# HDaoud/ORBSLAMM

Measured on AMD Instinct MI355X. Metric: frames/s ORB extract+match, 1241x376 @2000 kp; bit-exact kp/desc vs CPU, higher is better.
Workload: dtype u8

## Files before the change

### orbslamm_amd/csrc/orbx_geometry.inc

```

static int init_tables(orbx_handle* h)
{
    const OrbxParams& p = h->prm;
    if (p.nlevels < 1 || p.nlevels > ORBX_MAXL || p.nfeatures < 1 || !(p.scaleFactor > 1.0f))
        return fail(ORBX_E_INVALID, "bad ORBextractor parameters");
    const int L = p.nlevels;
    h->nlevels = L;
    const double scaleFactor = (double)p.scaleFactor;
    h->mvScaleFactor[0] = 1.0f;
    h->mvLevelSigma2[0] = 1.0f;
    for (int i = 1; i < L; i++) {
        h->mvScaleFactor[i] = (float)((double)h->mvScaleFactor[i - 1] * scaleFactor);
        h->mvLevelSigma2[i] = h->mvScaleFactor[i] * h->mvScaleFactor[i];
    }
    for (int i = 0; i < L; i++) {
        h->mvInvScaleFactor[i] = 1.0f / h->mvScaleFactor[i];
        h->mvInvLevelSigma2[i] = 1.0f / h->mvLevelSigma2[i];
    }
    const float factor = (float)(1.0 / scaleFactor);
    float nDesired = (float)p.nfeatures * (1 - factor) / (1 - (float)pow((double)factor, (double)L));
    int sum = 0;
    for (int l = 0; l < L - 1; l++) {
        h->mnFeaturesPerLevel[l] = cv_round(nDesired);
        sum += h->mnFeaturesPerLevel[l];
// ... 19 lines not shown
    Geom g;
    std::vector<Cell> cells;
    std::vector<short4> tabs;
    int xoff[ORBX_MAXL], yoff[ORBX_MAXL];
    int tileStrideDw, tileRows, fastListCap, tileRows0, fastListCap0, fastSmapPitch, fastSmapPitch0, nodeCap;
    BlurTiles bt;
    BlurRuns br;
    KpBlocks kb;
    int kbTotal;
    std::vector<PyrRange> pyrRanges;
    int pyrBlocks, pyrBufA, pyrBufB, pyrTabCap;
    bool pyrFused;
};

static inline size_t pyr_lds_bytes(int bufA, int bufB, int tabCap) { return ((size_t)bufA + bufB) * 4 + (size_t)tabCap * 16; }

static int build_geometry(const orbx_handle* h, int w, int h0, HostGeom& out)
{
    Geom& g = out.g;
    memset(&g, 0, sizeof g);
    g.nlevels = h->nlevels;
    g.w0 = w; g.h0 = h0;
    g.iniTh = h->prm.iniThFAST; g.minTh = h->prm.minThFAST;
    memcpy(g.umax, h->umax, sizeof g.umax);
    if (w > 8191 || h0 > 8191) return fail(ORBX_E_UNSUPPORTED, "frame larger than 8191 px");
    out.cells.clear();
    out.tabs.clear();
    int pyrOff = 0, blurOff = 0, candOff = 0, keptOff = 0, maxRoiW = 8, maxRoiH = 8, maxRoiW0 = 8, maxRoiH0 = 8, nodeCap = 16, maxCells = 1;
    for (int l = 0; l < g.nlevels; l++) {
        LevelGeom& L = g.lv[l];
// ... 249 lines not shown
```

### orbslamm_amd/csrc/orbx_kernels.hip

```cpp
#include <hip/hip_runtime.h>
#include <stdint.h>

#include "orbx_common.hpp"

namespace orbx {

struct FrameSrc {
    const uint8_t* img0;
    int32_t stride0;
    int64_t pitch0;
    uint8_t* pyr;
    uint8_t* blur;
    int32_t f0;
};

__device__ __forceinline__ const uint8_t* level_ptr(const Geom* g, const FrameSrc& s, int f, int l, int& stride)
{
    if (l == 0) { stride = s.stride0; return s.img0 + (int64_t)f * s.pitch0; }
    stride = g->lv[l].stride;
    return s.pyr + (int64_t)f * g->pyrFrameBytes + g->lv[l].pyrOff;
}

__device__ __forceinline__ bool xcd_block_frame(int nframes, int& blk, int& fr)
{
// ... 1551 lines not shown
constexpr DiscItems make_disc_items()
{
    DiscItems d{};
    int n = 0;
    for (int r = 0; r <= 2 * kDiscR; r++) {
        const int ay = r < kDiscR ? kDiscR - r : r - kDiscR, h = kDiscHalf[ay];
        for (int c = (kDiscR - h) / 4; c <= (kDiscR + h) / 4; c++) d.rc[n++] = (uint16_t)(r << 4 | c);
    }
    d.n = n;
    for (int t = n; t < kDiscLoads * 64; t++) d.rc[t] = d.rc[n - 1];
    return d;
}
__device__ const DiscItems kDisc = make_disc_items();
static_assert(make_disc_items().n <= kDiscLoads * 64 && make_disc_items().n > (kDiscLoads - 1) * 64, "five loads, not four");

__global__ __launch_bounds__(256) void k_orient_desc(const Geom* __restrict__ g, FrameSrc src, KpBlocks kb,
                                                    const uint64_t* __restrict__ kept,
                                                    const int32_t* __restrict__ keptCount,
                                                    OrbxKeyPointDev* __restrict__ outKps,
                                                    uint8_t* __restrict__ outDesc, int32_t* __restrict__ outCount, int nframes,
                                                    uint8_t* __restrict__ outX, int64_t xPitch, int64_t xAngOff)
{
#if ORBX_DESC_PRIO
    __builtin_amdgcn_s_setprio(ORBX_DESC_PRIO);
#endif
#ifdef ORBX_ORIENT_TIMING
    uint64_t ts[10]; int nts = 0;
#define OSTAMP() ts[nts++] = wall_clock64()
#else
#define OSTAMP() do {} while (0)
#endif
    OSTAMP();
    __shared__ float4 spat[256];
    __shared__ uint32_t swu[256], sw1[256];
    constexpr int PR = kDiscR, PDW = 10, PROWS = 2 * PR + 1;
    __shared__ uint32_t spatch[kKpPerBlock][PROWS * PDW];
    const int tid = threadIdx.x, lane = tid & 63, wave = tid >> 6;
    const int q = lane >> 4, ql = lane & 15;
    int bx, fr;
    if (!xcd_block_frame(nframes, bx, fr)) return;
    const int f = fr + src.f0;
    int l = 0;
    while (l + 1 < g->nlevels && bx >= kb.base[l + 1]) l++;
    const int idx = (bx - kb.base[l]) * kKpPerBlock + wave * 4 + q;
    const int nl = g->nlevels;
    const LevelGeom& L = g->lv[l];
    const uint64_t rec0 = kept[(int64_t)f * g->keptFrameRecs + L.keptOff + idx];
    int32_t pk = ((const int32_t*)d_pattern)[tid];
    const int tv = (tid >> 3) - kHalfPatch;
    int um = g->umax[(tv < 0 ? -tv : tv) & 15];
    int before = 0, totalAll = 0, mine = 0;
    for (int i = 0; i < nl; i++) {
        const int c = keptCount[f * nl + i];
        if (i < l) before += c;
        if (i == l) mine = c;
        totalAll += c;
    }
    if (bx == 0 && tid == 0) outCount[f] = totalAll < g->maxKp ? totalAll : g->maxKp;
    int ditem[kDiscLoads];
#pragma unroll
    for (int i = 0; i < kDiscLoads; i++) ditem[i] = kDisc.rc[64 * i + lane];
    asm volatile("" : "+v"(pk), "+v"(um), "+v"(ditem[0]), "+v"(ditem[1]), "+v"(ditem[2]), "+v"(ditem[3]), "+v"(ditem[4]));
    static_assert(kDiscLoads == 5, "operand list above");
    const int o = before + idx;
    const bool active = idx < mine && o < g->maxKp;
    const bool anyActive = __builtin_amdgcn_ballot_w64(active) != 0;
    OSTAMP();
    const uint64_t rec = active ? rec0 : 0;
    const int cx = (int)cand_x(rec) + kMinBorder, cy = (int)cand_y(rec) + kMinBorder;
    int stride;
    const uint8_t* img = level_ptr(g, src, f, l, stride);
    const int bs = L.blurStride;
    const uint8_t* blur = src.blur + (int64_t)f * g->blurFrameBytes + L.blurOff;
    const int ctrOff = cy * stride + cx, bctrOff = cy * bs + cx;

    OSTAMP();
    uint32_t dw[4][4];
    if (anyActive) {
        const uint32_t voff = (uint32_t)((lane >> 3) * stride + 4 * (lane & 7));
#pragma unroll
        for (int k = 0; k < 4; k++) {
            const uint8_t* pk = img + (__builtin_amdgcn_readlane(ctrOff, 16 * k) - kHalfPatch * stride - 16);
#pragma unroll
            for (int j = 0; j < 4; j++) gload_sbase(dw[k][j], voff, pk + 8 * j * stride);
        }
    }
    constexpr int NPI = kDiscLoads;
    uint32_t pd[4][NPI];
    int sidx[NPI];
    if (anyActive) {
        uint32_t voff[NPI];
#pragma unroll
        for (int i = 0; i < NPI; i++) {
            const int it = ditem[i], r = it >> 4, c = it & 15;
            voff[i] = (uint32_t)(r * bs + 4 * c);
            sidx[i] = r * PDW + c;
        }
#pragma unroll
        for (int k = 0; k < 4; k++) {
            const int so = __builtin_amdgcn_readlane((int)active, 16 * k) ? __builtin_amdgcn_readlane(bctrOff, 16 * k) : __builtin_amdgcn_readlane(bctrOff, 0);
            const uint8_t* pk = blur + (so - PR * bs - PR);
#pragma unroll
            for (int i = 0; i < NPI; i++) gload_sbase(pd[k][i], voff[i], pk);
        }
    }
    {
        spat[tid] = make_float4((float)(int8_t)(pk & 0xFF), (float)(int8_t)((pk >> 8) & 0xFF),
                                (float)(int8_t)((pk >> 16) & 0xFF), (float)(int8_t)((pk >> 24) & 0xFF));
        const int u0 = 4 * (tid & 7) - 16;
        const int d = tid < 248 ? um : -1;
        uint32_t wu = 0, w1 = 0;
#pragma unroll
        for (int j = 0; j < 4; j++) {
            const int u = u0 + j;
            if (u >= -d && u <= d) { wu |= (uint32_t)(u + 16) << (8 * j); w1 |= 1u << (8 * j); }
        }
        swu[tid] = wu; sw1[tid] = w1;
    }
    __syncthreads();
    if (!anyActive) return;
    OSTAMP();
    int m10, m01;
    asm volatile("s_waitcnt vmcnt(20)"
                 : "+v"(dw[0][0]), "+v"(dw[0][1]), "+v"(dw[0][2]), "+v"(dw[0][3]), "+v"(dw[1][0]), "+v"(dw[1][1]), "+v"(dw[1][2]), "+v"(dw[1][3]),
                   "+v"(dw[2][0]), "+v"(dw[2][1]), "+v"(dw[2][2]), "+v"(dw[2][3]), "+v"(dw[3][0]), "+v"(dw[3][1]), "+v"(dw[3][2]), "+v"(dw[3][3]));
    static_assert(4 * NPI == 20, "vmcnt above");
    {
        int A[4], B[4];
        uint32_t wu[4], w1[4], wv[4];
#pragma unroll
        for (int j = 0; j < 4; j++) {
            wu[j] = swu[lane + 64 * j];
            w1[j] = sw1[lane + 64 * j];
            wv[j] = w1[j] * (uint32_t)(8 * j + (lane >> 3) + 1);
        }
#pragma unroll
        for (int k = 0; k < 4; k++) {
            uint32_t su = 0, sv = 0, s1 = 0;
#pragma unroll
            for (int j = 0; j < 4; j++) {
                su = __builtin_amdgcn_udot4(dw[k][j], wu[j], su, false);
                sv = __builtin_amdgcn_udot4(dw[k][j], wv[j], sv, false);
                s1 = __builtin_amdgcn_udot4(dw[k][j], w1[j], s1, false);
            }
            A[k] = (int)su - 16 * (int)s1;
            B[k] = (int)sv - 16 * (int)s1;
        }
        auto swap32 = [](int a, int b) { const auto r = __builtin_amdgcn_permlane32_swap((unsigned)a, (unsigned)b, false, false); return (int)(r[0] + r[1]); };
        auto swap16 = [](int a, int b) { const auto r = __builtin_amdgcn_permlane16_swap((unsigned)a, (unsigned)b, false, false); return (int)(r[0] + r[1]); };
        m10 = swap16(swap32(A[0], A[2]), swap32(A[1], A[3]));
        m01 = swap16(swap32(B[0], B[2]), swap32(B[1], B[3]));
        m10 += __builtin_amdgcn_update_dpp(0, m10, 0x128, 0xF, 0xF, false);
        m01 += __builtin_amdgcn_update_dpp(0, m01, 0x128, 0xF, 0xF, false);
        m10 += __builtin_amdgcn_update_dpp(0, m10, 0x124, 0xF, 0xF, false);
        m01 += __builtin_amdgcn_update_dpp(0, m01, 0x124, 0xF, 0xF, false);
        m10 += __builtin_amdgcn_update_dpp(0, m10, 0x122, 0xF, 0xF, false);
        m01 += __builtin_amdgcn_update_dpp(0, m01, 0x122, 0xF, 0xF, false);
        m10 += __builtin_amdgcn_update_dpp(0, m10, 0x121, 0xF, 0xF, false);
        m01 += __builtin_amdgcn_update_dpp(0, m01, 0x121, 0xF, 0xF, false);
    }
    OSTAMP();
    asm volatile("s_waitcnt vmcnt(0)"
                 : "+v"(pd[0][0]), "+v"(pd[0][1]), "+v"(pd[0][2]), "+v"(pd[0][3]), "+v"(pd[0][4]),
                   "+v"(pd[1][0]), "+v"(pd[1][1]), "+v"(pd[1][2]), "+v"(pd[1][3]), "+v"(pd[1][4]),
                   "+v"(pd[2][0]), "+v"(pd[2][1]), "+v"(pd[2][2]), "+v"(pd[2][3]), "+v"(pd[2][4]),
                   "+v"(pd[3][0]), "+v"(pd[3][1]), "+v"(pd[3][2]), "+v"(pd[3][3]), "+v"(pd[3][4]));
    static_assert(NPI == 5, "operand list above");
#pragma unroll
    for (int k = 0; k < 4; k++)
#pragma unroll
        for (int i = 0; i < NPI; i++) spatch[wave * 4 + k][sidx[i]] = pd[k][i];
    const float angle = fast_atan2_deg((float)m01, (float)m10);

    constexpr float factorPI = (float)(3.1415926535897932384626433832795 / 180.f);
    const float ang = __fmul_rn(angle, factorPI);
    float a, b;
    orbx_sincosf_0_2pi(ang, &b, &a);
    OSTAMP();
    const uint8_t* const sp8 = (const uint8_t*)&spatch[0][0];
    constexpr float kRnd = 12582912.f;
    const uint32_t adj = (uint32_t)((wave * 4 + q) * (PROWS * PDW * 4) + PR * (PDW * 4) + PR) - 0x400000u * (uint32_t)(PDW * 4) - 0x4B400000u;
    static_assert(PDW * 4 == 40, "row pitch is an inline constant of the mad below");
    uint32_t myWord = 0;
    typedef float f2v __attribute__((ext_vector_type(2)));
    const f2v AB = {a, b}, KR = {kRnd, kRnd};
    auto rot = [&](const f2v p, int& rx, int& ry) {
        f2v U, V, W, Z;
        asm("v_pk_mul_f32 %0, %1, %2 op_sel:[0,0] op_sel_hi:[0,1]" : "=v"(U) : "v"(p), "v"(AB));
        asm("v_pk_mul_f32 %0, %1, %2 op_sel:[1,1] op_sel_hi:[1,0] neg_lo:[0,1]" : "=v"(V) : "v"(p), "v"(AB));
        asm("v_pk_add_f32 %0, %1, %2" : "=v"(W) : "v"(U), "v"(V));
        asm("v_pk_add_f32 %0, %1, %2" : "=v"(Z) : "v"(W), "v"(KR));
        rx = __float_as_int(Z.x); ry = __float_as_int(Z.y);
    };
#pragma unroll
    for (int t = 0; t < 16; t++) {
        const float4 pt = spat[ql + 16 * t];
        int rx0, ry0, rx1, ry1;
        rot(f2v{pt.x, pt.y}, rx0, ry0);
        rot(f2v{pt.z, pt.w}, rx1, ry1);
        uint32_t o0, o1;
        asm("v_mad_i32_i24 %0, %1, 40, %2" : "=v"(o0) : "v"(ry0), "v"(rx0));
        asm("v_mad_i32_i24 %0, %1, 40, %2" : "=v"(o1) : "v"(ry1), "v"(rx1));
        const int t0 = sp8[o0 + adj], t1 = sp8[o1 + adj];
        const uint64_t bal = __builtin_amdgcn_ballot_w64(t0 < t1);
        const uint32_t w16 = (uint32_t)(bal >> (16 * q)) & 0xFFFFu;
        if (ql == t) myWord = w16;
    }
    OSTAMP();
#ifdef ORBX_ORIENT_TIMING
    if (lane == 0 && wave == 0 && fr == 0 && (bx % 29) == 0)
        printf("ORIENT bx %d l %d: barrier %.2f counts %.2f rec %.2f moments %.2f trig %.2f brief %.2f us\n", bx, l, (ts[1]-ts[0])/100.0, (ts[2]-ts[1])/100.0, (ts[3]-ts[2])/100.0, (ts[4]-ts[3])/100.0, (ts[5]-ts[4])/100.0, (ts[6]-ts[5])/100.0);
#endif
    if (outX) {
        uint16_t* const sw = (uint16_t*)&spatch[wave * 4 + q][0];
        sw[ql] = (uint16_t)myWord;
        __builtin_amdgcn_fence(__ATOMIC_RELEASE, "wavefront");
        __builtin_amdgcn_wave_barrier();
        __builtin_amdgcn_fence(__ATOMIC_ACQUIRE, "wavefront");
        const int kq = (lane >> 3) & 3, c = lane & 7;
        const int oq = __shfl(o, 16 * kq);
        const bool aq = __shfl((int)active, 16 * kq) != 0;
        if (lane < 32 && aq) {
            const uint32_t bits = spatch[wave * 4 + kq][c];
            auto pm1 = [](uint32_t b8) {
                uint32_t x = (b8 | (b8 << 12)) & 0x000F000Fu;
                x = (x | (x << 6)) & 0x03030303u;
                x = (x | (x << 3)) & 0x11111111u;
                return 0x22222222u | ((x ^ 0x11111111u) << 3);
            };
            const uint4 e = make_uint4(pm1(bits & 255), pm1((bits >> 8) & 255), pm1((bits >> 16) & 255), pm1(bits >> 24));
            *(uint4*)(outX + (int64_t)f * xPitch + (int64_t)(oq >> 5) * 4096 + (int64_t)(c * 32 + (oq & 31)) * 16) = e;
        }
    }
    if (active) {
        ((uint16_t*)(outDesc + ((int64_t)f * g->maxKp + o) * 32))[ql] = (uint16_t)myWord;
        if (ql == 1 && outX) *(float*)(outX + (int64_t)f * xPitch + xAngOff + (int64_t)o * 4) = angle;
        if (ql == 0) {
            OrbxKeyPointDev kp;
            kp.x = __fmul_rn((float)cx, L.scale);
            kp.y = __fmul_rn((float)cy, L.scale);
            kp.size = L.kpSize;
            kp.angle = angle;
            kp.response = (float)cand_resp(rec);
            kp.octave = l;
            kp.class_id = -1;
            outKps[(int64_t)f * g->maxKp + o] = kp;
        }
    }
}

__global__ __launch_bounds__(256) void k_upload(const uint4* __restrict__ src, uint4* __restrict__ dst, int n16)
{
    typedef unsigned int u32x4 __attribute__((ext_vector_type(4)));
    const int i = blockIdx.x * 256 + threadIdx.x;
    if (i < n16) ((u32x4*)dst)[i] = __builtin_nontemporal_load((const u32x4*)src + i);
}

struct UploadSrcs { const uint4* src[8]; };
__global__ __launch_bounds__(256) void k_upload_frames(UploadSrcs s, uint4* __restrict__ dst, int n16)
{
    typedef unsigned int u32x4 __attribute__((ext_vector_type(4)));
    const int i = blockIdx.x * 256 + threadIdx.x, f = blockIdx.y;
// ... 220 lines not shown
```

### orbslamm_amd/csrc/orbx_pipeline.inc

```

static int configure_shape(orbx_handle* h, int w, int hh)
{
    if (h->curW == w && h->curH == hh) return ORBX_OK;
    if (w > h->maxW || hh > h->maxH) return fail(ORBX_E_INVALID, "frame %dx%d exceeds the handle's maximum %dx%d", w, hh, h->maxW, h->maxH);
    HostGeom hg;
    int rc = build_geometry(h, w, hh, hg);
    if (rc) return rc;
    if (hg.cells.size() > h->cellsCap || hg.tabs.size() > h->tabsCap || (size_t)hg.g.pyrFrameBytes > h->pyrCapFrame ||
        (size_t)hg.g.blurFrameBytes > h->blurCapFrame || (size_t)hg.g.candFrameRecs > h->candCapFrame ||
        (size_t)hg.g.keptFrameRecs > h->keptCapFrame || hg.g.maxKp > h->maxKp)
        return fail(ORBX_E_INVALID, "frame %dx%d needs more scratch than the handle was created with", w, hh);
    const size_t dl = dist_lds_bytes(hg.nodeCap, hg.g.maxCellsPerLevel);
    h->distInLds = dl <= 156 * 1024;
    if (h->distInLds && dl > 48 * 1024 &&
        hipFuncSetAttribute((const void*)k_distribute<true>, hipFuncAttributeMaxDynamicSharedMemorySize, (int)dl) != hipSuccess) {
        (void)hipGetLastError();
        h->distInLds = false;
    }
    if (h->distInLds) {
        h->distBlurOk = hipFuncSetAttribute((const void*)k_distribute_blur, hipFuncAttributeMaxDynamicSharedMemorySize, (int)dl) == hipSuccess;
        if (!h->distBlurOk) (void)hipGetLastError();
    } else {
        const size_t need = dl * (size_t)h->maxB * hg.g.nlevels;
        if (need > h->distScratchBytes && ((rc = sync_all(h)) || (rc = regrow_exact(h->d_distScratch, h->distScratchBytes, need, need)))) return rc;
// ... 102 lines not shown
        if (!h->distInLds || !h->distBlurOk || h->prof.cur || src.f0 != 0) return false;
        const size_t dl = dist_lds_bytes(h->nodeCap, g.maxCellsPerLevel);
        const int nTiles = h->blurTiles.base[g.nlevels];
        DistArgs da{h->d_geom, h->d_candRaw, h->d_candA, h->d_candB, h->d_cells, h->d_cellCount, h->d_candCount, h->d_kept, h->d_keptCount,
                    h->d_errCur, h->nodeCap, src.f0, nullptr, 0, 0};
        hipLaunchKernelGGL(k_distribute_blur, dim3(g.nlevels + (nTiles + 1) / 2, nb), dim3(kDistThreads), dl, s, da, src, h->blurTiles, nTiles);
        return true;
    }
    void blur(hipStream_t s, bool lat = false) const
    {
        h->prof.begin(P_BLUR, s);
        if (lat) hipLaunchKernelGGL(k_blur_mfma, dim3(h->blurTiles.base[h->geom.nlevels], xcd_grid_y(nb)), dim3(256), 0, s, h->d_geom, src, h->blurTiles, nb);
        else hipLaunchKernelGGL(k_blur_walk, dim3(h->blurRuns.base[h->geom.nlevels], xcd_grid_y(nb)), dim3(256), 0, s, h->d_geom, src, h->blurRuns, nb);
        h->prof.end(s);
    }
    int desc(hipStream_t s, int set, hipEvent_t done = nullptr) const
    {
        if (h->matchPending[set] && h->matchStream[set] != s) HIPCHK(hipStreamWaitEvent(s, h->evMatch[set], 0));
        if (h->evOutOfSet[set] && h->outStream[set] != s) HIPCHK(hipStreamWaitEvent(s, h->evOutOfSet[set], 0));
        for (hipEvent_t e : h->evExtReader[set]) HIPCHK(hipStreamWaitEvent(s, e, 0));
        h->evExtReader[set].clear();
        uint8_t* const xOut = h->fuseExpand ? r_xdesc(h, set) + (size_t)h->xPitch : nullptr;
        return launch_done(h, P_ORIENT_DESC, k_orient_desc, dim3(h->kpBlocksTotal, xcd_grid_y(nb)), dim3(256), 0, s, done, h->d_geom, src, h->kpBlocks, h->d_kept,
                           h->d_keptCount, r_kps(h, set) + h->maxKp, r_desc(h, set) + (size_t)h->maxKp * 32, r_count(h, set) + 1, nb, xOut, h->xPitch, h->xAngOff);
    }
};

struct FrameRange { int f0, f1; };
static inline FrameRange part_range(int B, int part, int nparts) { return {(int)((int64_t)B * part / nparts), (int)((int64_t)B * (part + 1) / nparts)}; }
struct CallMode { bool lat; int parts; };
static inline CallMode call_mode(const orbx_handle* h, int B)
{
    const bool lat = B <= h->latMaxB && !h->serial;
    return {lat, lat || h->serial ? 1 : std::min(h->nsplit, B)};
}

static int run_extract(orbx_handle* h, const uint8_t* d_imgs, int B, int w, int hh, int stride, size_t pitch,
                       const hipEvent_t* evUploaded = nullptr, hipStream_t sIn = nullptr, bool lazyDone = false)
{
// ... 44 lines not shown
            }
        } else {
            if (evFrames && sIn != sm) HIPCHK(hipStreamWaitEvent(sm, evFrames, 0));
            if (evFrames && sIn != sa) HIPCHK(hipStreamWaitEvent(sa, evFrames, 0));
            if (sIn == sa && h->partEverRan[0]) { if ((rc = flush_part_event(h))) return rc; HIPCHK(hipStreamWaitEvent(sa, h->evPart[0], 0)); }
            L.fast(sa, 0, cellsL0);
            L.dist(sa, 0, 1);
            if ((rc = L.pyramid(sm, h->evPyr[0]))) return rc;
            L.fast(sm, cellsL0, g.totalCells - cellsL0);
            L.dist(sm, 1, g.nlevels - 1);
            HIPCHK(hipStreamWaitEvent(sa, h->evPyr[0], 0));
            L.blur(sa, true);
            HIPCHK(hipEventRecord(h->evFast0[0], sa));
            HIPCHK(hipStreamWaitEvent(sm, h->evFast0[0], 0));
        }
        if ((rc = L.desc(sm, set, lazyDone ? nullptr : h->evPart[0]))) return rc;
        h->lastParts = 1; h->partLazy = lazyDone; h->partEverRan[0] = true;
    } else {
        for (int part = 0; part < nsplit; part++) {
            const FrameRange fr = part_range(B, part, nsplit);
            const int f0 = fr.f0, nb = fr.f1 - fr.f0;
            if (nb <= 0) continue;
            hipStream_t s = h->serial ? s0 : h->streamP[part];
            hipStream_t s2 = h->serial ? s : s0;
            if (evUploaded) {
                HIPCHK(hipStreamWaitEvent(s, evUploaded[part], 0));
                if (s2 != s) HIPCHK(hipStreamWaitEvent(s2, evUploaded[part], 0));
            }
            if (evFrames && !h->serial) HIPCHK(hipStreamWaitEvent(s, evFrames, 0));
            if (evFrames && !h->serial && sIn != s0 && part == 0) HIPCHK(hipStreamWaitEvent(s0, evFrames, 0));
            src.f0 = f0;
// ... 3 lines not shown
                if (h->partEverRan[part]) HIPCHK(hipStreamWaitEvent(s2, h->evPart[part], 0));
                L.fast(s2, 0, cellsL0);
                HIPCHK(hipEventRecord(h->evFast0[part], s2));
            } else {
                L.fast(s, 0, cellsL0);
            }
            if ((rc = L.pyramid(s))) return rc;
            HIPCHK(hipEventRecord(h->evPyr[part], s));
            HIPCHK(hipStreamWaitEvent(s2, h->evPyr[part], 0));
            L.blur(s2, B <= h->latMaxB);
            HIPCHK(hipEventRecord(h->evBlur[part], s2));
            L.fast(s, cellsL0, g.totalCells - cellsL0);
            if (splitFast) HIPCHK(hipStreamWaitEvent(s, h->evFast0[part], 0));
            L.dist(s, 0, g.nlevels);
            HIPCHK(hipStreamWaitEvent(s, h->evBlur[part], 0));
            if ((rc = L.desc(s, set))) return rc;
            HIPCHK(hipEventRecord(h->evPart[h->lastParts++], s));
            h->partEverRan[part] = true;
        }
    }
    HIPCHK(hipGetLastError());
    h->lastB = B;
    src.f0 = 0;
    h->lastSrc = src;
    return ORBX_OK;
}

extern "C" int orbx_extract_batch_device(orbx_t* h, const uint8_t* d_imgs, int B, int w, int hh, int stride, size_t pitch)
{
    int rc = check_device(h);
    if (rc) return rc;
// ... 81 lines not shown
```

### orbslamm_amd/csrc/orbx_probe.inc

```

extern "C" int orbx_compute_stereo_matches(orbx_t* left, orbx_t* right, int frame, float mb, float mbf,
                                           float* u_right, float* depth, int cap, int* n_left)
{
    int rc = orbx_sync(right);
    if (rc) return rc;
    if ((rc = orbx_sync(left))) return rc;
    if (left->device != right->device) return fail(ORBX_E_INVALID, "the two extractors live on different devices");
    if (left->curW == 0 || left->curW != right->curW || left->curH != right->curH || left->nlevels != right->nlevels)
        return fail(ORBX_E_INVALID, "left and right frames differ in shape or pyramid");
    if (frame < 0 || frame >= left->lastB || frame >= right->lastB) return fail(ORBX_E_INVALID, "frame %d not in the last batches", frame);
    if (!(mb > 0.f) || !(mbf > 0.f)) return fail(ORBX_E_INVALID, "stereo baseline (mb, mbf) must be positive");
    if (left->maxKp >= 65536 || right->maxKp >= 65536) return fail(ORBX_E_UNSUPPORTED, "more than 65535 keypoints per frame");
    int32_t n = 0;
    HIPCHK(hipMemcpy(&n, r_count(left, left->curSet) + 1 + frame, sizeof n, hipMemcpyDeviceToHost));
    if (n_left) *n_left = n;
    if (n > cap) return fail(ORBX_E_CAPACITY, "%d keypoints, caller capacity %d", n, cap);
    if (n == 0) return ORBX_OK;
    const size_t need = (size_t)left->maxKp * 12 + 64;
    if (need > left->stereoBytes && (rc = regrow_exact(left->d_stereo, left->stereoBytes, need, need))) return rc;
    StereoArgs a;
    a.kL = r_kps(left, left->curSet) + (size_t)(frame + 1) * left->maxKp; a.dL = r_desc(left, left->curSet) + (size_t)(frame + 1) * left->maxKp * 32;
    a.nL = r_count(left, left->curSet) + 1 + frame;
    a.kR = r_kps(right, right->curSet) + (size_t)(frame + 1) * right->maxKp; a.dR = r_desc(right, right->curSet) + (size_t)(frame + 1) * right->maxKp * 32;
    a.nR = r_count(right, right->curSet) + 1 + frame;
// ... 180 lines not shown
    auto launch = [&](int k, hipStream_t s) {
        switch (k) {
        case 0: (void)L.pyramid(s); break;
        case 1: L.fast(s, 0, cellsL0); L.fast(s, cellsL0, g.totalCells - cellsL0); break;
        case 2: L.dist(s, 0, g.nlevels); break;
        case 3: L.blur(s); break;
        case 4: (void)L.desc(s, set); break;
        default: match_kernels(h, s, set, nb, 0.7f, 50, 1); break;
        }
    };
    if (lds_bytes && wg_threads && wgs) {
        const size_t pl = pyr_lds_bytes(h->pyrBufA, h->pyrBufB, h->pyrTabCap);
        const size_t fl = fast_lds_bytes(h->tileRows, h->tileStrideDw, h->fastSmapPitch, h->fastListCap);
        const int nqb = (h->maxKp + orbm::kMfmaRowsPerBlock - 1) / orbm::kMfmaRowsPerBlock;
        const int32_t l[K] = {(int32_t)pl, (int32_t)fl, (int32_t)(dist_lds_bytes(h->nodeCap, g.maxCellsPerLevel) + 5552), (kBlurWalkInWords + kBlurMfmaOutWords) * 4, 31104, orbm::kMfmaLdsBytes};
        const int32_t t[K] = {256, 64, kDistThreads, 256, 256, 256};
        const int32_t w[K] = {h->pyrBlocks * nb, g.totalCells * nb, g.nlevels * nb, h->blurRuns.base[g.nlevels] * nb, h->kpBlocksTotal * nb, nqb * nb};
        for (int k = 0; k < K; k++) { lds_bytes[k] = l[k]; wg_threads[k] = t[k]; wgs[k] = w[k]; }
    }
    for (int k = 0; k < K; k++) if (names) names[k] = kNames[k];
    hipStream_t sa = h->streamP[0], sb = h->streamP[1];
    hipEvent_t e0, e1, eGo;
    HIPCHK(hipEventCreate(&e0)); HIPCHK(hipEventCreate(&e1)); HIPCHK(hipEventCreateWithFlags(&eGo, hipEventDisableTiming));
    auto timed = [&](int i, int j, int ni, int nj, float& ms) -> int {
        HIPCHK(hipEventRecord(eGo, h->stream));
        HIPCHK(hipStreamWaitEvent(sa, eGo, 0));
        if (j >= 0) { HIPCHK(hipStreamWaitEvent(sb, eGo, 0)); for (int r = 0; r < nj / 4; r++) launch(j, sb); }
        HIPCHK(hipEventRecord(e0, sa));
        for (int r = 0; r < ni; r++) { launch(i, sa); if (j >= 0) for (int q = 0; q * ni < nj - nj / 4 && q < 8; q++) launch(j, sb); }
        HIPCHK(hipEventRecord(e1, sa));
        HIPCHK(hipStreamSynchronize(sa)); HIPCHK(hipStreamSynchronize(sb));
// ... 24 lines not shown
```

### orbslamm_amd/csrc/orbx_streams.inc

```

struct ChainPool { hipStream_t s[4] = {nullptr, nullptr, nullptr, nullptr}; int users[4] = {0, 0, 0, 0}; bool made = false; };
static ChainPool g_chain[64];
static std::mutex g_chainMu;

static bool chain_prio_normal() { static const bool v = env_char("ORBX_LAT_PRIO") == '0'; return v; }

static int chain_stream_acquire(int device, int priority, hipStream_t* out, int* idx)
{
    std::lock_guard<std::mutex> lk(g_chainMu);
    ChainPool& cp = g_chain[device & 63];
    if (!cp.made) {
        hipStream_t s[4] = {nullptr, nullptr, nullptr, nullptr};
        void* scratch = nullptr;
        hipError_t e = hipMalloc(&scratch, 256);
        for (int i = 0; i < 4 && e == hipSuccess; i++) e = hipStreamCreateWithPriority(&s[i], hipStreamNonBlocking, priority);
        for (int i = 0; i < 4 && e == hipSuccess; i++) { e = hipMemsetAsync(scratch, 0, 256, s[i]); if (e == hipSuccess) e = hipStreamSynchronize(s[i]); }
        if (scratch) (void)hipFree(scratch);
        if (e != hipSuccess) {
            for (hipStream_t st : s) if (st) (void)hipStreamDestroy(st);
            return fail(ORBX_E_HIP, "cannot make the chain streams of device %d: %s", device, hipGetErrorString(e));
        }
        for (int i = 0; i < 4; i++) cp.s[i] = s[i];
        cp.made = true;
    }
// ... 160 lines not shown
        HIPCHK_OR(new_event(h, h->evBlur[i]), undo());
        HIPCHK_OR(new_event(h, h->evPart[i]), undo());
        HIPCHK_OR(new_event(h, h->evFast0[i]), undo());
    }
    HIPCHK_OR(new_event(h, h->evStart), undo());
    for (int i = 0; i < 2; i++) { HIPCHK_OR(new_event(h, h->evMatch[i]), undo()); HIPCHK_OR(new_event(h, h->evMatched[i]), undo()); }
    const size_t B = (size_t)max_batch;
    h->cellsCap = hg.cells.size() * 2 + 64;
    h->tabsCap = hg.tabs.size() * 2 + 64;
    h->imgFrameBytes = (size_t)align_up(max_w, 64) * max_h;
    h->pyrCapFrame = (size_t)hg.g.pyrFrameBytes + 4096;
    h->blurCapFrame = (size_t)hg.g.blurFrameBytes + 4096;
    h->candCapFrame = (size_t)hg.g.candFrameRecs + 1024;
    h->keptCapFrame = (size_t)hg.g.keptFrameRecs + 64;
    h->maxKp = hg.g.maxKp + 64;
    HIPCHK_OR(dev_alloc(h, h->d_geom, sizeof(Geom)), undo());
    HIPCHK_OR(dev_alloc(h, h->d_cells, h->cellsCap * sizeof(Cell)), undo());
    HIPCHK_OR(dev_alloc(h, h->d_tabs, h->tabsCap * sizeof(short4)), undo());
    h->pyrRangesCap = 64 * ORBX_MAXL;
    HIPCHK_OR(hipMalloc(&h->d_pyrRanges, h->pyrRangesCap * sizeof(PyrRange)), undo());
    HIPCHK_OR(dev_alloc(h, h->d_pyr, h->pyrCapFrame * B), undo());
    HIPCHK_OR(dev_alloc(h, h->d_blur, h->blurCapFrame * B), undo());
    HIPCHK_OR(dev_alloc(h, h->d_candRaw, h->candCapFrame * B * sizeof(uint64_t)), undo());
    HIPCHK_OR(dev_alloc(h, h->d_candA, h->candCapFrame * B * sizeof(uint64_t)), undo());
    HIPCHK_OR(dev_alloc(h, h->d_candB, h->candCapFrame * B * sizeof(uint64_t)), undo());
    HIPCHK_OR(dev_alloc(h, h->d_candCount, B * ORBX_MAXL * sizeof(int32_t)), undo());
    HIPCHK_OR(dev_alloc(h, h->d_cellCount, B * h->cellsCap * sizeof(int32_t)), undo());
    HIPCHK_OR(dev_alloc(h, h->d_kept, h->keptCapFrame * B * sizeof(uint64_t)), undo());
    HIPCHK_OR(dev_alloc(h, h->d_keptCount, B * ORBX_MAXL * sizeof(int32_t)), undo());
    HIPCHK_OR(dev_alloc(h, h->d_err, 8 * sizeof(int32_t)), undo());
    HIPCHK_OR(dev_alloc(h, h->d_kps, 2 * (B + 1) * h->maxKp * sizeof(OrbxKeyPointDev)), undo());
// ... 78 lines not shown
```

Before: 188,700.

## Template orient/desc kernel to process eight keypoints per wave for batched paths

```diff
diff --git a/orbslamm_amd/csrc/orbx_geometry.inc b/orbslamm_amd/csrc/orbx_geometry.inc
--- a/orbslamm_amd/csrc/orbx_geometry.inc
+++ b/orbslamm_amd/csrc/orbx_geometry.inc
@@ -57,6 +57,24 @@
 };
 
 static inline size_t pyr_lds_bytes(int bufA, int bufB, int tabCap) { return ((size_t)bufA + bufB) * 4 + (size_t)tabCap * 16; }
+
+static const int8_t kPatternHost[1024] = {
+#include "brief_pattern.inc"
+};
+static void build_orient_tables(const int umax[16], OrientTables& t)
+{
+    for (int i = 0; i < 256; i++) {
+        t.spat[i] = make_float4((float)kPatternHost[4 * i], (float)kPatternHost[4 * i + 1], (float)kPatternHost[4 * i + 2], (float)kPatternHost[4 * i + 3]);
+        const int v = (i >> 3) - kHalfPatch, u0 = 4 * (i & 7) - 16;
+        const int d = i < 248 ? umax[(v < 0 ? -v : v) & 15] : -1;
+        uint32_t wu = 0, w1 = 0;
+        for (int j = 0; j < 4; j++) {
+            const int u = u0 + j;
+            if (u >= -d && u <= d) { wu |= (uint32_t)(u + 16) << (8 * j); w1 |= 1u << (8 * j); }
+        }
+        t.swu[i] = wu; t.sw1[i] = w1;
+    }
+}
 
 static int build_geometry(const orbx_handle* h, int w, int h0, HostGeom& out)
 {
diff --git a/orbslamm_amd/csrc/orbx_kernels.hip b/orbslamm_amd/csrc/orbx_kernels.hip
--- a/orbslamm_amd/csrc/orbx_kernels.hip
+++ b/orbslamm_amd/csrc/orbx_kernels.hip
@@ -1589,13 +1589,22 @@
 __device__ const DiscItems kDisc = make_disc_items();
 static_assert(make_disc_items().n <= kDiscLoads * 64 && make_disc_items().n > (kDiscLoads - 1) * 64, "five loads, not four");
 
-__global__ __launch_bounds__(256) void k_orient_desc(const Geom* __restrict__ g, FrameSrc src, KpBlocks kb,
+struct OrientTables { float4 spat[256]; uint32_t swu[256], sw1[256]; };
+static_assert(sizeof(Geom) % 16 == 0 && sizeof(OrientTables) == 6144, "the tables follow the Geom block, 16-byte aligned");
+__device__ __forceinline__ const OrientTables* orient_tables(const Geom* g) { return (const OrientTables*)(g + 1); }
+
+template <int KPW>
+__global__ __launch_bounds__(kKpPerBlock / KPW * 64) void k_orient_desc(const Geom* __restrict__ g, FrameSrc src, KpBlocks kb,
                                                     const uint64_t* __restrict__ kept,
                                                     const int32_t* __restrict__ keptCount,
                                                     OrbxKeyPointDev* __restrict__ outKps,
                                                     uint8_t* __restrict__ outDesc, int32_t* __restrict__ outCount, int nframes,
                                                     uint8_t* __restrict__ outX, int64_t xPitch, int64_t xAngOff)
 {
+    static_assert(KPW == 4 || KPW == 8, "a quarter or an eighth of the wave per keypoint");
+    constexpr int EL = 64 / KPW, ELSH = KPW == 4 ? 4 : 3;
+    constexpr int NT = kKpPerBlock / KPW * 64;
+    static_assert(NT == 256 || (KPW == 8 && NT == 128), "the tables' 256 entries are built by 256 threads, or copied by 128 or 256");
 #if ORBX_DESC_PRIO
     __builtin_amdgcn_s_setprio(ORBX_DESC_PRIO);
 #endif
@@ -1611,19 +1620,34 @@
     constexpr int PR = kDiscR, PDW = 10, PROWS = 2 * PR + 1;
     __shared__ uint32_t spatch[kKpPerBlock][PROWS * PDW];
     const int tid = threadIdx.x, lane = tid & 63, wave = tid >> 6;
-    const int q = lane >> 4, ql = lane & 15;
+    const int q = lane >> ELSH, ql = lane & (EL - 1);
     int bx, fr;
     if (!xcd_block_frame(nframes, bx, fr)) return;
     const int f = fr + src.f0;
     int l = 0;
     while (l + 1 < g->nlevels && bx >= kb.base[l + 1]) l++;
-    const int idx = (bx - kb.base[l]) * kKpPerBlock + wave * 4 + q;
+    const int idx = (bx - kb.base[l]) * kKpPerBlock + wave * KPW + q;
     const int nl = g->nlevels;
     const LevelGeom& L = g->lv[l];
     const uint64_t rec0 = kept[(int64_t)f * g->keptFrameRecs + L.keptOff + idx];
-    int32_t pk = ((const int32_t*)d_pattern)[tid];
-    const int tv = (tid >> 3) - kHalfPatch;
-    int um = g->umax[(tv < 0 ? -tv : tv) & 15];
+    int32_t pk = 0;
+    int um = 0;
+    float4 tp0, tp1;
+    uint2 twu, tw1;
+    if constexpr (KPW == 4) {
+        pk = ((const int32_t*)d_pattern)[tid];
+        const int tv = (tid >> 3) - kHalfPatch;
+        um = g->umax[(tv < 0 ? -tv : tv) & 15];
+    } else {
+        const OrientTables* const T = orient_tables(g);
+        if constexpr (NT == 128) {
+            tp0 = T->spat[tid]; tp1 = T->spat[tid + 128];
+            twu = ((const uint2*)T->swu)[tid]; tw1 = ((const uint2*)T->sw1)[tid];
+        } else {
+            tp0 = tp1 = T->spat[tid];
+            twu.x = twu.y = T->swu[tid]; tw1.x = tw1.y = T->sw1[tid];
+        }
+    }
     int before = 0, totalAll = 0, mine = 0;
     for (int i = 0; i < nl; i++) {
         const int c = keptCount[f * nl + i];
@@ -1635,8 +1659,14 @@
     int ditem[kDiscLoads];
 #pragma unroll
     for (int i = 0; i < kDiscLoads; i++) ditem[i] = kDisc.rc[64 * i + lane];
-    asm volatile("" : "+v"(pk), "+v"(um), "+v"(ditem[0]), "+v"(ditem[1]), "+v"(ditem[2]), "+v"(ditem[3]), "+v"(ditem[4]));
-    static_assert(kDiscLoads == 5, "operand list above");
+    if constexpr (KPW == 4) {
+        asm volatile("" : "+v"(pk), "+v"(um), "+v"(ditem[0]), "+v"(ditem[1]), "+v"(ditem[2]), "+v"(ditem[3]), "+v"(ditem[4]));
+    } else {
+        asm volatile("" : "+v"(tp0.x), "+v"(tp0.y), "+v"(tp0.z), "+v"(tp0.w), "+v"(tp1.x), "+v"(tp1.y), "+v"(tp1.z), "+v"(tp1.w),
+                          "+v"(twu.x), "+v"(twu.y), "+v"(tw1.x), "+v"(tw1.y),
+                          "+v"(ditem[0]), "+v"(ditem[1]), "+v"(ditem[2]), "+v"(ditem[3]), "+v"(ditem[4]));
+    }
+    static_assert(kDiscLoads == 5, "operand lists above");
     const int o = before + idx;
     const bool active = idx < mine && o < g->maxKp;
     const bool anyActive = __builtin_amdgcn_ballot_w64(active) != 0;
@@ -1650,18 +1680,18 @@
     const int ctrOff = cy * stride + cx, bctrOff = cy * bs + cx;
 
     OSTAMP();
-    uint32_t dw[4][4];
+    uint32_t dw[KPW][4];
     if (anyActive) {
         const uint32_t voff = (uint32_t)((lane >> 3) * stride + 4 * (lane & 7));
 #pragma unroll
-        for (int k = 0; k < 4; k++) {
-            const uint8_t* pk = img + (__builtin_amdgcn_readlane(ctrOff, 16 * k) - kHalfPatch * stride - 16);
+        for (int k = 0; k < KPW; k++) {
+            const uint8_t* pk = img + (__builtin_amdgcn_readlane(ctrOff, EL * k) - kHalfPatch * stride - 16);
 #pragma unroll
             for (int j = 0; j < 4; j++) gload_sbase(dw[k][j], voff, pk + 8 * j * stride);
         }
     }
     constexpr int NPI = kDiscLoads;
-    uint32_t pd[4][NPI];
+    uint32_t pd[KPW][NPI];
     int sidx[NPI];
     if (anyActive) {
         uint32_t voff[NPI];
@@ -1672,14 +1702,14 @@
             sidx[i] = r * PDW + c;
         }
 #pragma unroll
-        for (int k = 0; k < 4; k++) {
-            const int so = __builtin_amdgcn_readlane((int)active, 16 * k) ? __builtin_amdgcn_readlane(bctrOff, 16 * k) : __builtin_amdgcn_readlane(bctrOff, 0);
+        for (int k = 0; k < KPW; k++) {
+            const int so = __builtin_amdgcn_readlane((int)active, EL * k) ? __builtin_amdgcn_readlane(bctrOff, EL * k) : __builtin_amdgcn_readlane(bctrOff, 0);
             const uint8_t* pk = blur + (so - PR * bs - PR);
 #pragma unroll
             for (int i = 0; i < NPI; i++) gload_sbase(pd[k][i], voff[i], pk);
         }
     }
-    {
+    if constexpr (KPW == 4) {
         spat[tid] = make_float4((float)(int8_t)(pk & 0xFF), (float)(int8_t)((pk >> 8) & 0xFF),
                                 (float)(int8_t)((pk >> 16) & 0xFF), (float)(int8_t)((pk >> 24) & 0xFF));
         const int u0 = 4 * (tid & 7) - 16;
@@ -1691,17 +1721,33 @@
             if (u >= -d && u <= d) { wu |= (uint32_t)(u + 16) << (8 * j); w1 |= 1u << (8 * j); }
         }
         swu[tid] = wu; sw1[tid] = w1;
+    } else {
+        if constexpr (NT == 128) {
+            spat[tid] = tp0; spat[tid + 128] = tp1;
+            ((uint2*)swu)[tid] = twu; ((uint2*)sw1)[tid] = tw1;
+        } else {
+            spat[tid] = tp0; swu[tid] = twu.x; sw1[tid] = tw1.x;
+        }
     }
     __syncthreads();
     if (!anyActive) return;
     OSTAMP();
     int m10, m01;
-    asm volatile("s_waitcnt vmcnt(20)"
-                 : "+v"(dw[0][0]), "+v"(dw[0][1]), "+v"(dw[0][2]), "+v"(dw[0][3]), "+v"(dw[1][0]), "+v"(dw[1][1]), "+v"(dw[1][2]), "+v"(dw[1][3]),
-                   "+v"(dw[2][0]), "+v"(dw[2][1]), "+v"(dw[2][2]), "+v"(dw[2][3]), "+v"(dw[3][0]), "+v"(dw[3][1]), "+v"(dw[3][2]), "+v"(dw[3][3]));
-    static_assert(4 * NPI == 20, "vmcnt above");
+    if constexpr (KPW == 4) {
+        asm volatile("s_waitcnt vmcnt(20)"
+                     : "+v"(dw[0][0]), "+v"(dw[0][1]), "+v"(dw[0][2]), "+v"(dw[0][3]), "+v"(dw[1][0]), "+v"(dw[1][1]), "+v"(dw[1][2]), "+v"(dw[1][3]),
+                       "+v"(dw[2][0]), "+v"(dw[2][1]), "+v"(dw[2][2]), "+v"(dw[2][3]), "+v"(dw[3][0]), "+v"(dw[3][1]), "+v"(dw[3][2]), "+v"(dw[3][3]));
+    } else {
+        asm volatile("s_waitcnt vmcnt(40)"
+                     : "+v"(dw[0][0]), "+v"(dw[0][1]), "+v"(dw[0][2]), "+v"(dw[0][3]), "+v"(dw[1][0]), "+v"(dw[1][1]), "+v"(dw[1][2]), "+v"(dw[1][3]),
+                       "+v"(dw[2][0]), "+v"(dw[2][1]), "+v"(dw[2][2]), "+v"(dw[2][3]), "+v"(dw[3][0]), "+v"(dw[3][1]), "+v"(dw[3][2]), "+v"(dw[3][3]));
+        asm volatile(""
+                     : "+v"(dw[4][0]), "+v"(dw[4][1]), "+v"(dw[4][2]), "+v"(dw[4][3]), "+v"(dw[5][0]), "+v"(dw[5][1]), "+v"(dw[5][2]), "+v"(dw[5][3]),
+                       "+v"(dw[6][0]), "+v"(dw[6][1]), "+v"(dw[6][2]), "+v"(dw[6][3]), "+v"(dw[7][0]), "+v"(dw[7][1]), "+v"(dw[7][2]), "+v"(dw[7][3]));
+    }
+    static_assert(4 * NPI == 20 && 8 * NPI == 40, "vmcnt above");
     {
-        int A[4], B[4];
+        int A[KPW], B[KPW];
         uint32_t wu[4], w1[4], wv[4];
 #pragma unroll
         for (int j = 0; j < 4; j++) {
@@ -1710,7 +1756,7 @@
             wv[j] = w1[j] * (uint32_t)(8 * j + (lane >> 3) + 1);
         }
 #pragma unroll
-        for (int k = 0; k < 4; k++) {
+        for (int k = 0; k < KPW; k++) {
             uint32_t su = 0, sv = 0, s1 = 0;
 #pragma unroll
             for (int j = 0; j < 4; j++) {
@@ -1723,28 +1769,55 @@
         }
         auto swap32 = [](int a, int b) { const auto r = __builtin_amdgcn_permlane32_swap((unsigned)a, (unsigned)b, false, false); return (int)(r[0] + r[1]); };
         auto swap16 = [](int a, int b) { const auto r = __builtin_amdgcn_permlane16_swap((unsigned)a, (unsigned)b, false, false); return (int)(r[0] + r[1]); };
-        m10 = swap16(swap32(A[0], A[2]), swap32(A[1], A[3]));
-        m01 = swap16(swap32(B[0], B[2]), swap32(B[1], B[3]));
-        m10 += __builtin_amdgcn_update_dpp(0, m10, 0x128, 0xF, 0xF, false);
-        m01 += __builtin_amdgcn_update_dpp(0, m01, 0x128, 0xF, 0xF, false);
-        m10 += __builtin_amdgcn_update_dpp(0, m10, 0x124, 0xF, 0xF, false);
-        m01 += __builtin_amdgcn_update_dpp(0, m01, 0x124, 0xF, 0xF, false);
-        m10 += __builtin_amdgcn_update_dpp(0, m10, 0x122, 0xF, 0xF, false);
-        m01 += __builtin_amdgcn_update_dpp(0, m01, 0x122, 0xF, 0xF, false);
-        m10 += __builtin_amdgcn_update_dpp(0, m10, 0x121, 0xF, 0xF, false);
-        m01 += __builtin_amdgcn_update_dpp(0, m01, 0x121, 0xF, 0xF, false);
+        if constexpr (KPW == 4) {
+            m10 = swap16(swap32(A[0], A[2]), swap32(A[1], A[3]));
+            m01 = swap16(swap32(B[0], B[2]), swap32(B[1], B[3]));
+            m10 += __builtin_amdgcn_update_dpp(0, m10, 0x128, 0xF, 0xF, false);
+            m01 += __builtin_amdgcn_update_dpp(0, m01, 0x128, 0xF, 0xF, false);
+            m10 += __builtin_amdgcn_update_dpp(0, m10, 0x124, 0xF, 0xF, false);
+            m01 += __builtin_amdgcn_update_dpp(0, m01, 0x124, 0xF, 0xF, false);
+            m10 += __builtin_amdgcn_update_dpp(0, m10, 0x122, 0xF, 0xF, false);
+            m01 += __builtin_amdgcn_update_dpp(0, m01, 0x122, 0xF, 0xF, false);
+            m10 += __builtin_amdgcn_update_dpp(0, m10, 0x121, 0xF, 0xF, false);
+            m01 += __builtin_amdgcn_update_dpp(0, m01, 0x121, 0xF, 0xF, false);
+        } else {
+            const int e10 = swap16(swap32(A[0], A[4]), swap32(A[2], A[6])), o10 = swap16(swap32(A[1], A[5]), swap32(A[3], A[7]));
+            const int e01 = swap16(swap32(B[0], B[4]), swap32(B[2], B[6])), o01 = swap16(swap32(B[1], B[5]), swap32(B[3], B[7]));
+            const bool odd = (lane & 8) != 0;
+            m10 = (odd ? o10 : e10) + __builtin_amdgcn_update_dpp(0, odd ? e10 : o10, 0x128, 0xF, 0xF, false);
+            m01 = (odd ? o01 : e01) + __builtin_amdgcn_update_dpp(0, odd ? e01 : o01, 0x128, 0xF, 0xF, false);
+            m10 += __builtin_amdgcn_update_dpp(0, m10, 0x141, 0xF, 0xF, false);
+            m01 += __builtin_amdgcn_update_dpp(0, m01, 0x141, 0xF, 0xF, false);
+            m10 += __builtin_amdgcn_update_dpp(0, m10, 0xB1, 0xF, 0xF, false);
+            m01 += __builtin_amdgcn_update_dpp(0, m01, 0xB1, 0xF, 0xF, false);
+            m10 += __builtin_amdgcn_update_dpp(0, m10, 0x4E, 0xF, 0xF, false);
+            m01 += __builtin_amdgcn_update_dpp(0, m01, 0x4E, 0xF, 0xF, false);
+        }
     }
     OSTAMP();
-    asm volatile("s_waitcnt vmcnt(0)"
-                 : "+v"(pd[0][0]), "+v"(pd[0][1]), "+v"(pd[0][2]), "+v"(pd[0][3]), "+v"(pd[0][4]),
-                   "+v"(pd[1][0]), "+v"(pd[1][1]), "+v"(pd[1][2]), "+v"(pd[1][3]), "+v"(pd[1][4]),
-                   "+v"(pd[2][0]), "+v"(pd[2][1]), "+v"(pd[2][2]), "+v"(pd[2][3]), "+v"(pd[2][4]),
-                   "+v"(pd[3][0]), "+v"(pd[3][1]), "+v"(pd[3][2]), "+v"(pd[3][3]), "+v"(pd[3][4]));
-    static_assert(NPI == 5, "operand list above");
-#pragma unroll
-    for (int k = 0; k < 4; k++)
-#pragma unroll
-        for (int i = 0; i < NPI; i++) spatch[wave * 4 + k][sidx[i]] = pd[k][i];
+    if constexpr (KPW == 4) {
+        asm volatile("s_waitcnt vmcnt(0)"
+                     : "+v"(pd[0][0]), "+v"(pd[0][1]), "+v"(pd[0][2]), "+v"(pd[0][3]), "+v"(pd[0][4]),
+                       "+v"(pd[1][0]), "+v"(pd[1][1]), "+v"(pd[1][2]), "+v"(pd[1][3]), "+v"(pd[1][4]),
+                       "+v"(pd[2][0]), "+v"(pd[2][1]), "+v"(pd[2][2]), "+v"(pd[2][3]), "+v"(pd[2][4]),
+                       "+v"(pd[3][0]), "+v"(pd[3][1]), "+v"(pd[3][2]), "+v"(pd[3][3]), "+v"(pd[3][4]));
+    } else {
+        asm volatile("s_waitcnt vmcnt(0)"
+                     : "+v"(pd[0][0]), "+v"(pd[0][1]), "+v"(pd[0][2]), "+v"(pd[0][3]), "+v"(pd[0][4]),
+                       "+v"(pd[1][0]), "+v"(pd[1][1]), "+v"(pd[1][2]), "+v"(pd[1][3]), "+v"(pd[1][4]),
+                       "+v"(pd[2][0]), "+v"(pd[2][1]), "+v"(pd[2][2]), "+v"(pd[2][3]), "+v"(pd[2][4]),
+                       "+v"(pd[3][0]), "+v"(pd[3][1]), "+v"(pd[3][2]), "+v"(pd[3][3]), "+v"(pd[3][4]));
+        asm volatile(""
+                     : "+v"(pd[4][0]), "+v"(pd[4][1]), "+v"(pd[4][2]), "+v"(pd[4][3]), "+v"(pd[4][4]),
+                       "+v"(pd[5][0]), "+v"(pd[5][1]), "+v"(pd[5][2]), "+v"(pd[5][3]), "+v"(pd[5][4]),
+                       "+v"(pd[6][0]), "+v"(pd[6][1]), "+v"(pd[6][2]), "+v"(pd[6][3]), "+v"(pd[6][4]),
+                       "+v"(pd[7][0]), "+v"(pd[7][1]), "+v"(pd[7][2]), "+v"(pd[7][3]), "+v"(pd[7][4]));
+    }
+    static_assert(NPI == 5, "operand lists above");
+#pragma unroll
+    for (int k = 0; k < KPW; k++)
+#pragma unroll
+        for (int i = 0; i < NPI; i++) spatch[wave * KPW + k][sidx[i]] = pd[k][i];
     const float angle = fast_atan2_deg((float)m01, (float)m10);
 
     constexpr float factorPI = (float)(3.1415926535897932384626433832795 / 180.f);
@@ -1754,7 +1827,7 @@
     OSTAMP();
     const uint8_t* const sp8 = (const uint8_t*)&spatch[0][0];
     constexpr float kRnd = 12582912.f;
-    const uint32_t adj = (uint32_t)((wave * 4 + q) * (PROWS * PDW * 4) + PR * (PDW * 4) + PR) - 0x400000u * (uint32_t)(PDW * 4) - 0x4B400000u;
+    const uint32_t adj = (uint32_t)((wave * KPW + q) * (PROWS * PDW * 4) + PR * (PDW * 4) + PR) - 0x400000u * (uint32_t)(PDW * 4) - 0x4B400000u;
     static_assert(PDW * 4 == 40, "row pitch is an inline constant of the mad below");
     uint32_t myWord = 0;
     typedef float f2v __attribute__((ext_vector_type(2)));
@@ -1767,9 +1840,11 @@
         asm("v_pk_add_f32 %0, %1, %2" : "=v"(Z) : "v"(W), "v"(KR));
         rx = __float_as_int(Z.x); ry = __float_as_int(Z.y);
     };
-#pragma unroll
-    for (int t = 0; t < 16; t++) {
-        const float4 pt = spat[ql + 16 * t];
+    [[maybe_unused]] const uint32_t balShift = 8 * (q & 3);
+    [[maybe_unused]] uint32_t collect = 0;
+#pragma unroll
+    for (int t = 0; t < 256 / EL; t++) {
+        const float4 pt = spat[ql + EL * t];
         int rx0, ry0, rx1, ry1;
         rot(f2v{pt.x, pt.y}, rx0, ry0);
         rot(f2v{pt.z, pt.w}, rx1, ry1);
@@ -1778,49 +1853,69 @@
         asm("v_mad_i32_i24 %0, %1, 40, %2" : "=v"(o1) : "v"(ry1), "v"(rx1));
         const int t0 = sp8[o0 + adj], t1 = sp8[o1 + adj];
         const uint64_t bal = __builtin_amdgcn_ballot_w64(t0 < t1);
-        const uint32_t w16 = (uint32_t)(bal >> (16 * q)) & 0xFFFFu;
-        if (ql == t) myWord = w16;
+        if constexpr (KPW == 4) {
+            const uint32_t w16 = (uint32_t)(bal >> (16 * q)) & 0xFFFFu;
+            if (ql == t) myWord = w16;
+        } else {
+            const uint32_t half = q >= 4 ? (uint32_t)(bal >> 32) : (uint32_t)bal;
+            collect |= ((half >> balShift) & 0xFFu) << (8 * (t & 3));
+            if ((t & 3) == 3) {
+                if (ql == (t >> 2)) myWord = collect;
+                collect = 0;
+            }
+        }
     }
     OSTAMP();
 #ifdef ORBX_ORIENT_TIMING
     if (lane == 0 && wave == 0 && fr == 0 && (bx % 29) == 0)
         printf("ORIENT bx %d l %d: barrier %.2f counts %.2f rec %.2f moments %.2f trig %.2f brief %.2f us\n", bx, l, (ts[1]-ts[0])/100.0, (ts[2]-ts[1])/100.0, (ts[3]-ts[2])/100.0, (ts[4]-ts[3])/100.0, (ts[5]-ts[4])/100.0, (ts[6]-ts[5])/100.0);
 #endif
-    if (outX) {
-        uint16_t* const sw = (uint16_t*)&spatch[wave * 4 + q][0];
-        sw[ql] = (uint16_t)myWord;
-        __builtin_amdgcn_fence(__ATOMIC_RELEASE, "wavefront");
-        __builtin_amdgcn_wave_barrier();
-        __builtin_amdgcn_fence(__ATOMIC_ACQUIRE, "wavefront");
-        const int kq = (lane >> 3) & 3, c = lane & 7;
-        const int oq = __shfl(o, 16 * kq);
-        const bool aq = __shfl((int)active, 16 * kq) != 0;
-        if (lane < 32 && aq) {
-            const uint32_t bits = spatch[wave * 4 + kq][c];
-            auto pm1 = [](uint32_t b8) {
-                uint32_t x = (b8 | (b8 << 12)) & 0x000F000Fu;
-                x = (x | (x << 6)) & 0x03030303u;
-                x = (x | (x << 3)) & 0x11111111u;
-                return 0x22222222u | ((x ^ 0x11111111u) << 3);
-            };
-            const uint4 e = make_uint4(pm1(bits & 255), pm1((bits >> 8) & 255), pm1((bits >> 16) & 255), pm1(bits >> 24));
-            *(uint4*)(outX + (int64_t)f * xPitch + (int64_t)(oq >> 5) * 4096 + (int64_t)(c * 32 + (oq & 31)) * 16) = e;
-        }
-    }
-    if (active) {
-        ((uint16_t*)(outDesc + ((int64_t)f * g->maxKp + o) * 32))[ql] = (uint16_t)myWord;
-        if (ql == 1 && outX) *(float*)(outX + (int64_t)f * xPitch + xAngOff + (int64_t)o * 4) = angle;
-        if (ql == 0) {
-            OrbxKeyPointDev kp;
-            kp.x = __fmul_rn((float)cx, L.scale);
-            kp.y = __fmul_rn((float)cy, L.scale);
-            kp.size = L.kpSize;
-            kp.angle = angle;
-            kp.response = (float)cand_resp(rec);
-            kp.octave = l;
-            kp.class_id = -1;
-            outKps[(int64_t)f * g->maxKp + o] = kp;
-        }
+    auto pm1 = [](uint32_t b8) {
+        uint32_t x = (b8 | (b8 << 12)) & 0x000F000Fu;
+        x = (x | (x << 6)) & 0x03030303u;
+        x = (x | (x << 3)) & 0x11111111u;
+        return 0x22222222u | ((x ^ 0x11111111u) << 3);
+    };
+    auto record = [&]() {
+        OrbxKeyPointDev kp;
+        kp.x = __fmul_rn((float)cx, L.scale);
+        kp.y = __fmul_rn((float)cy, L.scale);
+        kp.size = L.kpSize;
+        kp.angle = angle;
+        kp.response = (float)cand_resp(rec);
+        kp.octave = l;
+        kp.class_id = -1;
+        outKps[(int64_t)f * g->maxKp + o] = kp;
+    };
+    if constexpr (KPW == 4) {
+        if (outX) {
+            uint16_t* const sw = (uint16_t*)&spatch[wave * 4 + q][0];
+            sw[ql] = (uint16_t)myWord;
+            __builtin_amdgcn_fence(__ATOMIC_RELEASE, "wavefront");
+            __builtin_amdgcn_wave_barrier();
+            __builtin_amdgcn_fence(__ATOMIC_ACQUIRE, "wavefront");
+            const int kq = (lane >> 3) & 3, c = lane & 7;
+            const int oq = __shfl(o, 16 * kq);
+            const bool aq = __shfl((int)active, 16 * kq) != 0;
+            if (lane < 32 && aq) {
+                const uint32_t bits = spatch[wave * 4 + kq][c];
+                const uint4 e = make_uint4(pm1(bits & 255), pm1((bits >> 8) & 255), pm1((bits >> 16) & 255), pm1(bits >> 24));
+                *(uint4*)(outX + (int64_t)f * xPitch + (int64_t)(oq >> 5) * 4096 + (int64_t)(c * 32 + (oq & 31)) * 16) = e;
+            }
+        }
+        if (active) {
+            ((uint16_t*)(outDesc + ((int64_t)f * g->maxKp + o) * 32))[ql] = (uint16_t)myWord;
+            if (ql == 1 && outX) *(float*)(outX + (int64_t)f * xPitch + xAngOff + (int64_t)o * 4) = angle;
+            if (ql == 0) record();
+        }
+    } else if (active) {
+        if (outX) {
+            const uint4 e = make_uint4(pm1(myWord & 255), pm1((myWord >> 8) & 255), pm1((myWord >> 16) & 255), pm1(myWord >> 24));
+            *(uint4*)(outX + (int64_t)f * xPitch + (int64_t)(o >> 5) * 4096 + (int64_t)(ql * 32 + (o & 31)) * 16) = e;
+            if (ql == 1) *(float*)(outX + (int64_t)f * xPitch + xAngOff + (int64_t)o * 4) = angle;
+        }
+        ((uint32_t*)(outDesc + ((int64_t)f * g->maxKp + o) * 32))[ql] = myWord;
+        if (ql == 0) record();
     }
 }
 
diff --git a/orbslamm_amd/csrc/orbx_pipeline.inc b/orbslamm_amd/csrc/orbx_pipeline.inc
--- a/orbslamm_amd/csrc/orbx_pipeline.inc
+++ b/orbslamm_amd/csrc/orbx_pipeline.inc
@@ -140,15 +140,15 @@
         else hipLaunchKernelGGL(k_blur_walk, dim3(h->blurRuns.base[h->geom.nlevels], xcd_grid_y(nb)), dim3(256), 0, s, h->d_geom, src, h->blurRuns, nb);
         h->prof.end(s);
     }
-    int desc(hipStream_t s, int set, hipEvent_t done = nullptr) const
+    int desc(hipStream_t s, int set, hipEvent_t done = nullptr, bool lat = false) const
     {
         if (h->matchPending[set] && h->matchStream[set] != s) HIPCHK(hipStreamWaitEvent(s, h->evMatch[set], 0));
         if (h->evOutOfSet[set] && h->outStream[set] != s) HIPCHK(hipStreamWaitEvent(s, h->evOutOfSet[set], 0));
         for (hipEvent_t e : h->evExtReader[set]) HIPCHK(hipStreamWaitEvent(s, e, 0));
         h->evExtReader[set].clear();
         uint8_t* const xOut = h->fuseExpand ? r_xdesc(h, set) + (size_t)h->xPitch : nullptr;
-        return launch_done(h, P_ORIENT_DESC, k_orient_desc, dim3(h->kpBlocksTotal, xcd_grid_y(nb)), dim3(256), 0, s, done, h->d_geom, src, h->kpBlocks, h->d_kept,
-                           h->d_keptCount, r_kps(h, set) + h->maxKp, r_desc(h, set) + (size_t)h->maxKp * 32, r_count(h, set) + 1, nb, xOut, h->xPitch, h->xAngOff);
+        return launch_done(h, P_ORIENT_DESC, lat ? k_orient_desc<4> : k_orient_desc<8>, dim3(h->kpBlocksTotal, xcd_grid_y(nb)), dim3(kKpPerBlock / (lat ? 4 : 8) * 64), 0, s, done, h->d_geom, src,
+                           h->kpBlocks, h->d_kept, h->d_keptCount, r_kps(h, set) + h->maxKp, r_desc(h, set) + (size_t)h->maxKp * 32, r_count(h, set) + 1, nb, xOut, h->xPitch, h->xAngOff);
     }
 };
 
@@ -223,7 +223,7 @@
             HIPCHK(hipEventRecord(h->evFast0[0], sa));
             HIPCHK(hipStreamWaitEvent(sm, h->evFast0[0], 0));
         }
-        if ((rc = L.desc(sm, set, lazyDone ? nullptr : h->evPart[0]))) return rc;
+        if ((rc = L.desc(sm, set, lazyDone ? nullptr : h->evPart[0], true))) return rc;
         h->lastParts = 1; h->partLazy = lazyDone; h->partEverRan[0] = true;
     } else {
         for (int part = 0; part < nsplit; part++) {
@@ -257,7 +257,7 @@
             if (splitFast) HIPCHK(hipStreamWaitEvent(s, h->evFast0[part], 0));
             L.dist(s, 0, g.nlevels);
             HIPCHK(hipStreamWaitEvent(s, h->evBlur[part], 0));
-            if ((rc = L.desc(s, set))) return rc;
+            if ((rc = L.desc(s, set, nullptr, B <= h->latMaxB))) return rc;
             HIPCHK(hipEventRecord(h->evPart[h->lastParts++], s));
             h->partEverRan[part] = true;
         }
diff --git a/orbslamm_amd/csrc/orbx_probe.inc b/orbslamm_amd/csrc/orbx_probe.inc
--- a/orbslamm_amd/csrc/orbx_probe.inc
+++ b/orbslamm_amd/csrc/orbx_probe.inc
@@ -218,7 +218,7 @@
         const size_t fl = fast_lds_bytes(h->tileRows, h->tileStrideDw, h->fastSmapPitch, h->fastListCap);
         const int nqb = (h->maxKp + orbm::kMfmaRowsPerBlock - 1) / orbm::kMfmaRowsPerBlock;
         const int32_t l[K] = {(int32_t)pl, (int32_t)fl, (int32_t)(dist_lds_bytes(h->nodeCap, g.maxCellsPerLevel) + 5552), (kBlurWalkInWords + kBlurMfmaOutWords) * 4, 31104, orbm::kMfmaLdsBytes};
-        const int32_t t[K] = {256, 64, kDistThreads, 256, 256, 256};
+        const int32_t t[K] = {256, 64, kDistThreads, 256, kKpPerBlock / 8 * 64, 256};
         const int32_t w[K] = {h->pyrBlocks * nb, g.totalCells * nb, g.nlevels * nb, h->blurRuns.base[g.nlevels] * nb, h->kpBlocksTotal * nb, nqb * nb};
         for (int k = 0; k < K; k++) { lds_bytes[k] = l[k]; wg_threads[k] = t[k]; wgs[k] = w[k]; }
     }
diff --git a/orbslamm_amd/csrc/orbx_streams.inc b/orbslamm_amd/csrc/orbx_streams.inc
--- a/orbslamm_amd/csrc/orbx_streams.inc
+++ b/orbslamm_amd/csrc/orbx_streams.inc
@@ -198,7 +198,12 @@
     h->candCapFrame = (size_t)hg.g.candFrameRecs + 1024;
     h->keptCapFrame = (size_t)hg.g.keptFrameRecs + 64;
     h->maxKp = hg.g.maxKp + 64;
-    HIPCHK_OR(dev_alloc(h, h->d_geom, sizeof(Geom)), undo());
+    HIPCHK_OR(dev_alloc(h, h->d_geom, sizeof(Geom) + sizeof(OrientTables)), undo());
+    {
+        OrientTables ot;
+        build_orient_tables(h->umax, ot);
+        HIPCHK_OR(hipMemcpy(h->d_geom + 1, &ot, sizeof ot, hipMemcpyHostToDevice), undo());
+    }
     HIPCHK_OR(dev_alloc(h, h->d_cells, h->cellsCap * sizeof(Cell)), undo());
     HIPCHK_OR(dev_alloc(h, h->d_tabs, h->tabsCap * sizeof(short4)), undo());
     h->pyrRangesCap = 64 * ORBX_MAXL;
```

Result: faster. 193,600, median of 6 (+2.6%).
